# manyeyes/K2TransducerAsr

Hardware: AMD Instinct MI355X
Metric: RTFx (audio-sec/wall-sec) offline Zipformer greedy (higher is better)
Workload: dtype f32

## Files before the change

### k2transducerasr_amd/csrc/engine.cpp

```cpp
#include <cstring>
#include <thread>

#include "engine.h"
#include "lattice_ref.h"
#include "ctc_lattice_ref.h"
#include "kws_ref.h"
#include "ctc_prefix_bias_ref.h"
#include "ctc_prefix_ref.h"
#include "hotwords.h"
#include "ngram_lm.h"

#include <climits>
#include <cmath>

namespace k2hip {

namespace {
constexpr int kTailFrames = 19;
}

Engine::Engine(const std::string& weights, const char* overrides, int device) : device_(device) {
    tunables_init_from_env();
    model_.reset(new Model(weights, overrides));
    int n = 0;
// ... 233 lines not shown
    Arena& ar = *c.arena;
    const int D0 = m.cfg().dim[0];
    float* out = ar.take<float>((int64_t)B * T3 * D0);
    int64_t mark = ar.mark();
    float* a1 = ar.take<float>((int64_t)B * T1 * F0 * 8);
    conv0_swoosh(c, x, m.w("encoder_embed.conv.0.weight"), m.w("encoder_embed.conv.0.bias"), a1, B, T, F0);
    c.add_flops(0, 2.0 * B * T1 * (double)F0 * 8 * 9, 0);
    float* a2 = ar.take<float>((int64_t)B * T2 * F2 * 32);
    {
        GemmArgs g;
        g.A = a1; g.W = m.w("encoder_embed.conv.4.weight#ohwi"); g.ldw = 72; g.bias = m.w("encoder_embed.conv.4.bias");
        g.C = a2; g.ldc = 32; g.M = B * T2 * F2; g.N = 32; g.K = 72; g.act = ACT_SWOOSH_R;
        g.cv_Fout = F2; g.cv_Tout = T2; g.cv_Tin = T1; g.cv_Fin = F0; g.cv_C = 8; g.cv_st = 2; g.cv_sf = 2;
        g.seg_len = 24; g.seg_stride = F0 * 8;
        gemm(c, g);
    }
    float* a3 = ar.take<float>((int64_t)B * T3 * F3 * 128);
    {
        GemmArgs g;
        g.A = a2; g.W = m.w("encoder_embed.conv.7.weight#ohwi"); g.ldw = 288; g.bias = m.w("encoder_embed.conv.7.bias");
        g.C = a3; g.ldc = 128; g.M = B * T3 * F3; g.N = 128; g.K = 288; g.act = ACT_SWOOSH_R;
        g.cv_Fout = F3; g.cv_Tout = T3; g.cv_Tin = T2; g.cv_Fin = F2; g.cv_C = 32; g.cv_st = 1; g.cv_sf = 2;
        g.seg_len = 96; g.seg_stride = F2 * 32;
        gemm(c, g);
    }
    const int npix = B * T3 * F3;
    float* dw = ar.take<float>((int64_t)npix * 128);
    dwconv7x7(c, a3, m.w("encoder_embed.convnext.depthwise_conv.weight#kc"), m.w("encoder_embed.convnext.depthwise_conv.bias"),
              dw, B, T3, T3, 3, F3, 128);
    float* hid = ar.take<float>((int64_t)npix * 384);
    linear(c, dw, 128, m.w("encoder_embed.convnext.pointwise_conv1.weight"), m.w("encoder_embed.convnext.pointwise_conv1.bias"),
           hid, 384, npix, 128, 384, ACT_SWOOSH_L);
    linear(c, hid, 384, m.w("encoder_embed.convnext.pointwise_conv2.weight"), m.w("encoder_embed.convnext.pointwise_conv2.bias"),
           a3, 128, npix, 384, 128, ACT_NONE, a3, 128);
    float* lin = ar.take<float>((int64_t)B * T3 * D0);
    linear(c, a3, F3 * 128, m.w("encoder_embed.out.weight#fc"), m.w("encoder_embed.out.bias"), lin, D0, B * T3, F3 * 128, D0);
    biasnorm(c, lin, m.w("encoder_embed.out_norm.bias"), m.w("encoder_embed.out_norm.log_scale"), out, B * T3, D0);
    ar.rewind(mark);
    *T50 = T3;
    return out;
}

const float* Engine::pos_proj_cached(const Ctx& c, int layer, const float* pe, int pe_dim, const float* W, int rows, int ncols) {
    if (c.dry) return nullptr;
    std::lock_guard<std::mutex> lk(cache_mu_);
    const auto key = std::make_pair(layer, rows);
    auto it = pp_cache_.find(key);
// ... 68 lines not shown
    auto nonlin_attention = [&]() {
        if (site) {
            linear(c, src, D, w("nonlin_attention.in_proj.weight"), w("nonlin_attention.in_proj.bias"), hid, 3 * Hc, M, D, 3 * Hc);
            nonlin_av_out_ring(c, aw, ring(lay_.nonlin[gl]), hid, 3 * Hc, nullptr, nullptr, tmp2, B, T, KL, KLp, Hc, D);
        } else {
            GemmArgs g;
            g.A = aw; g.lda = KLp; g.sA0 = (long long)T * KLp;
            g.w_kn = 1;
            g.C = tmp2; g.ldc = Hc; g.sC0 = (long long)T * Hc;
            g.M = T; g.N = Hc; g.K = T; g.nb0 = B; g.nb1 = 1;
            if (M >= 256 && Hc % 16 == 0 && !tunables().no_glu_epilogue) {
                GemmArgs p;
                p.A = src; p.lda = D; p.W = w("nonlin_attention.in_proj.weight#glu"); p.ldw = D; p.bias = w("nonlin_attention.in_proj.bias#glu");
                p.C = hid; p.ldc = 2 * Hc; p.M = M; p.N = 3 * Hc; p.K = D; p.glu = 2; p.glu_cols = 2 * Hc;
                gemm(c, p);
                g.W = hid; g.ldw = 2 * Hc; g.sW0 = (long long)T * 2 * Hc;
                g.mul = hid + Hc; g.ldm = 2 * Hc; g.sM0 = (long long)T * 2 * Hc;
            } else {
                linear(c, src, D, w("nonlin_attention.in_proj.weight"), w("nonlin_attention.in_proj.bias"), hid, 3 * Hc, M, D, 3 * Hc);
                tanh_gate(c, hid, tmp, M, Hc);
                g.W = tmp; g.ldw = Hc; g.sW0 = (long long)T * Hc;
                g.mul = hid + 2 * Hc; g.ldm = 3 * Hc; g.sM0 = (long long)T * 3 * Hc;
            }
            gemm(c, g);
        }
        linear(c, tmp2, Hc, w("nonlin_attention.out_proj.weight"), w("nonlin_attention.out_proj.bias"), src, D, M, Hc, D, ACT_NONE, src, D);
    };
    auto self_attn = [&](int k) {
        const float *wi = wk("self_attn%d.in_proj.weight", k), *bi = wk("self_attn%d.in_proj.bias", k);
        const float *wo = wk("self_attn%d.out_proj.weight", k), *bo = wk("self_attn%d.out_proj.bias", k);
        if (vproj_fused) {
            attn_proj_av_out_ring(c, aw, ring(k == 1 ? lay_.val1[gl] : lay_.val2[gl]), src, wi, bi, wo, bo, src_alt, B, T, KL, KLp, H, vh, D);
            std::swap(src, src_alt);
            return;
        }
        linear(c, src, D, wi, bi, hid, HV, M, D, HV);
        if (site) {
            attn_av_out_ring(c, aw, ring(k == 1 ? lay_.val1[gl] : lay_.val2[gl]), hid, wo, bo, src, B, T, KL, KLp, H, vh, D);
            return;
        }
        if (attn_av_out(c, aw, hid, wo, bo, src, B, T, T, KLp, H, vh, D)) return;
        GemmArgs g;
        g.A = aw; g.lda = KLp; g.sA0 = (long long)T * KLp; g.sA1 = (long long)B * T * KLp;
        g.W = hid; g.w_kn = 1; g.ldw = HV; g.sW0 = (long long)T * HV; g.sW1 = vh;
        g.C = tmp; g.ldc = HV; g.sC0 = (long long)T * HV; g.sC1 = vh;
        g.M = T; g.N = vh; g.K = T; g.nb0 = B; g.nb1 = H;
        gemm(c, g);
// ... 1673 lines not shown
            const int ldh = I();
            float *wout = P(), *bias = P(), *x = P();
            const int B = I(), T = I(), KL = I(), Tp = I(), Hc = I(), D = I();
            nonlin_av_out_ring(c, aw, r, hid, ldh, wout, bias, x, B, T, KL, Tp, Hc, D);
        } else if (name == "attn_stream_ring" || name == "attn_stream") {
            float* qkp = P();
            const int ld = I();
            RingRef r;
            float* kcat = nullptr;
            if (name == "attn_stream_ring") r = ring(); else kcat = P();
            float* pp = P();
            const long long* plen = reinterpret_cast<const long long*>(P());
            float* aw = P();
            const int B = I(), Tc = I(), Lc = I(), KLp = I(), H = I(), ds = I(), left50 = I();
            if (kcat) attn_stream(c, qkp, ld, kcat, pp, plen, aw, B, Tc, Lc, KLp, H, ds, left50);
            else attn_stream_ring(c, qkp, ld, r, pp, plen, aw, B, Tc, Lc, KLp, H, ds, left50);
        } else if (name == "glu_causal_conv") {
            float *x2 = P(), *pool = P();
            const long long ss = L(), off = L();
            const int* slots = reinterpret_cast<const int*>(P());
            float *wc = P(), *bc = P(), *ww = P(), *bw = P(), *sc = P(), *y = P();
            const int B = I(), Tc = I(), D = I(), K = I();
            glu_causal_conv(c, x2, pool, ss, off, slots, wc, bc, ww, bw, sc, y, B, Tc, D, K);
        } else if (name == "gemm") {
            GemmArgs g;
            g.M = I(); g.N = I(); g.K = I();
            g.lda = I(); g.ldw = I(); g.ldc = I(); g.ldr = I();
            g.act = I(); g.act_cols = I(); g.w_kn = I();
            g.nb0 = I(); g.nb1 = I();
            g.sA0 = L(); g.sA1 = L(); g.sW0 = L(); g.sW1 = L(); g.sC0 = L(); g.sC1 = L(); g.sR0 = L(); g.sR1 = L();
            g.sBias0 = L();
            g.cv_Fout = I(); g.cv_Tout = I(); g.cv_Tin = I(); g.cv_Fin = I(); g.cv_C = I(); g.cv_st = I(); g.cv_sf = I();
            g.seg_len = I(); g.seg_stride = I();
            g.res_div = I(); g.act_after_res = I();
            g.glu = I(); g.glu_cols = I();
            g.ldm = I(); g.sM0 = L(); g.sM1 = L();
            g.ld_orig = I();
            const int cfg = I(), res_is_C = I();
            const long long oA = L(), oW = L(), oR = L(), oC = L(), oM = L(), oO = L();
            float *A = P(), *W = P(), *bias = P(), *res = P(), *C = P();
            const int* skip = reinterpret_cast<const int*>(P());
            float *mul = P(), *orig = P(), *scale = P();
            int* plan_out = reinterpret_cast<int*>(P());
            K2_REQUIRE(A && W && C && plan_out && buf_bytes[n_bufs - 1] >= 20, "debug_op_run gemm: A, W, C and a plan buffer of 5 ints are needed");
            K2_REQUIRE(!(res_is_C && res), "debug_op_run gemm: res_is_C takes no res buffer");
            K2_REQUIRE(oA >= 0 && oW >= 0 && oR >= 0 && oC >= 0 && oM >= 0 && oO >= 0, "debug_op_run gemm: negative offset");
            if (res_is_C) res = C;
            g.A = A + oA; g.W = W + oW; g.bias = bias; g.res = res ? res + oR : nullptr; g.C = C + oC;
            g.skip_if_zero = skip;
            g.mul = mul ? mul + oM : nullptr;
            g.byp_orig = orig ? orig + oO : nullptr; g.byp_scale = scale;
            GemmForceGuard force(cfg);
            const GemmPlan pl = plan_gemm(g, gemm_force());
            const int rep[5] = {(int)pl.family, pl.idx, pl.BM, pl.BN, pl.mode};
            K2_HIP(copy_blocking(plan_out, rep, sizeof rep, hipMemcpyHostToDevice));
            gemm(c, g);
        } else if (name == "gemm_glu_causal_conv") {
            float *x = P(), *wg = P(), *bg = P(), *pool = P();
            const long long ss = L(), off = L();
            const int* slots = reinterpret_cast<const int*>(P());
            float *wc = P(), *bc = P(), *ww = P(), *bw = P(), *sc = P(), *y = P();
            const int B = I(), Tc = I(), D = I(), K = I();
            int* entry_out = reinterpret_cast<int*>(P());
            K2_REQUIRE(entry_out && buf_bytes[n_bufs - 1] >= 4, "debug_op_run gemm_glu_causal_conv: an entry buffer of 1 int is needed");
            const int entry = glu_conv_ring_entry(B, Tc, D, K);
            K2_HIP(copy_blocking(entry_out, &entry, sizeof entry, hipMemcpyHostToDevice));
            took = gemm_glu_causal_conv(c, x, wg, bg, pool, ss, off, slots, wc, bc, ww, bw, sc, y, B, Tc, D, K);
        } else if (name == "biasnorm") {
            float *x = P(), *bias = P(), *ls = P(), *y = P();
            const int M = I(), D = I();
            biasnorm(c, x, bias, ls, y, M, D);
        } else if (name == "bypass") {
            float *orig = P(), *x = P(), *scale = P(), *y = P();
            const int M = I(), D = I();
            bypass(c, orig, x, scale, y, M, D);
        } else if (name == "biasnorm_bypass") {
            float *x = P(), *orig = P(), *nb = P(), *ls = P(), *scale = P(), *y = P();
            const int M = I(), D = I();
            biasnorm_bypass(c, x, orig, nb, ls, scale, y, M, D);
// ... 730 lines not shown
```

### k2transducerasr_amd/csrc/gemm.hip

```cpp
#include <algorithm>
#include <cmath>
#include <cstdlib>
#include <map>
#include <mutex>
#include <type_traits>

#include "act.h"
#include "kernels.h"

#pragma clang diagnostic ignored "-Winline-asm"

namespace k2hip {

typedef float f32x16 __attribute__((ext_vector_type(16)));
typedef float f32x4 __attribute__((ext_vector_type(4)));

namespace {


__device__ __forceinline__ float apply_act(float v, int act) {
    switch (act) {
        case ACT_SWOOSH_L: return swoosh_l(v);
        case ACT_SWOOSH_R: return swoosh_r(v);
        case ACT_TANH: {
// ... 481 lines not shown
            }
        }
    }

    K2_DMA_STAMP()
#pragma unroll
    for (int j = 0; j < NT; j++)
#pragma unroll
        for (int i = 0; i < MT; i++) {
            float vals[16];
#pragma unroll
            for (int r = 0; r < 16; r++) vals[r] = acc[i][j][r];
            epilogue_rows<16, Rows32>(g, vals, m0 + wr * WM + i * 32 + 4 * lh, n0 + wc * WN + j * 32 + li, C, nullptr, rres[i][j], R != nullptr,
                                      nullptr, g.bias ? g.bias + z0 * g.sBias0 : nullptr);
        }
    K2_DMA_STAMP()
    if (stamp && lane == 0) {
        stamp[62] = nstamp;
        stamp[63] = __builtin_amdgcn_s_memrealtime();
    }
#undef K2_DMA_STAMP
}

template <int BM, int BN, int WM, int WN, int NST>
__global__ __launch_bounds__(64 * (BM / WM) * (BN / WN)) void gemm_f32_mfma_pipe(GemmArgs g) {
    constexpr int BK = 32;
    constexpr int MT = WM / 32, NT = WN / 32;
    constexpr int WCOLS = BN / WN;
    constexpr int NW = (BM / WM) * (BN / WN);
    constexpr int NINST = (BM + BN) / 8;
    constexpr int IPW = NINST / NW;
    constexpr int STAGE = (BM + BN) * BK;
    constexpr int DPE = (IPW + 3) / 4;
    static_assert(NST == 3 || NST == 4, "pipe: three or four stages");
    static_assert(NINST % NW == 0, "pipe: every wave issues the same number of DMA instructions");
    static_assert((NST - 2) * IPW <= 63 && MT <= 4 && NT <= 2, "pipe: counted wait / wave tile out of range");

    if (g.skip_if_zero && *g.skip_if_zero == 0) return;
    extern __shared__ __attribute__((aligned(16))) float smem[];

    const int tid = threadIdx.x;
    const int lane = tid & 63, wave = __builtin_amdgcn_readfirstlane(tid >> 6);
    const int wr = wave / WCOLS, wc = wave % WCOLS;
    const int li = lane & 31, lh = lane >> 5;
    float* __restrict__ C = g.C;
    const float* __restrict__ R = g.res;
    int mb_, nb_;
    xcd_tile(mb_, nb_, g.xcd_panels == 1 ? 0 : g.M, g.N);
    const int m0 = mb_ * BM, n0 = nb_ * BN;
    const int nk = g.K / BK;

    unsigned long long* stamp = g.dbg ? g.dbg + ((size_t)(blockIdx.x + blockIdx.y * gridDim.x) * NW + wave) * 64 : nullptr;
    int nstamp = 0;
#define K2_PIPE_STAMP()                                                    \
    if (stamp) {  \
        if (lane == 0) stamp[nstamp] = __builtin_amdgcn_s_memtime();       \
        nstamp++;                                                          \
    }
    if (stamp && lane == 0) stamp[60] = __builtin_amdgcn_s_memrealtime();
    K2_PIPE_STAMP()

    const unsigned lds_base = (unsigned)(unsigned long long)(__attribute__((address_space(3))) char*)smem;
    unsigned voff[IPW];
    unsigned long long sb[IPW];
    unsigned mq[IPW];
#pragma unroll
    for (int q = 0; q < IPW; q++) {
        const int inst = wave + q * NW;
        const int slot = inst * 64 + lane;
        const int r = slot >> 3, cp = slot & 7;
        const int c = cp ^ ((r >> 1) & 7);
        const bool is_a = inst < BM / 8;
        const long long row = is_a ? min(m0 + r, g.M - 1) : min(n0 + (r - BM), g.N - 1);
        voff[q] = (unsigned)((row * (is_a ? g.lda : g.ldw) + 4 * c) * 4);
        const unsigned long long base = (unsigned long long)(is_a ? g.A : g.W);
        sb[q] = ((unsigned long long)(unsigned)__builtin_amdgcn_readfirstlane((int)(base >> 32)) << 32) |
                (unsigned long long)(unsigned)__builtin_amdgcn_readfirstlane((int)(unsigned)base);
        mq[q] = __builtin_amdgcn_readfirstlane(lds_base + inst * 1024);
    }

#define K2_PIPE_DMA(ST_, KT_, q_)                                                                                          \
    {                                                                                                                      \
        const unsigned long long src_ = sb[q_] + (unsigned long long)(KT_) * (BK * 4);                                    \
        asm volatile("s_add_u32 m0, %2, %3\n\ts_nop 0\n\tglobal_load_lds_dwordx4 %0, %1"                                    \
                     :                                                                                                     \
                     : "v"(voff[q_]), "s"(src_), "s"(mq[q_]), "n"((ST_) * STAGE * 4)                                       \
                     : "memory", "m0", "scc");                                                                                          \
    }
#define K2_PIPE_READ(SET_, ST_, G_)                                                                                        \
    {                                                                                                                      \
        _Pragma("unroll") for (int i = 0; i < MT; i++) fa[SET_][i] = *reinterpret_cast<const f32x4*>(ra[ST_][G_] + i * 32 * BK); \
        _Pragma("unroll") for (int j = 0; j < NT; j++) fb[SET_][j] = *reinterpret_cast<const f32x4*>(rb[ST_][G_] + j * 32 * BK); \
    }
#define K2_PIPE_FRAGS_READY(SET_) {}
#define K2_PIPE_STEP(ST_, KT_, HAS_NEXT_, DO_ISSUE_, WAIT_)                                                                \
    _Pragma("unroll") for (int gk = 0; gk < 4; gk++) {                                                                     \
        const int cu = gk & 1;                                                                                             \
        __builtin_amdgcn_sched_barrier(0);                                                                                 \
        K2_PIPE_FRAGS_READY(cu)                                                                                            \
        _Pragma("unroll") for (int e = 0; e < 4; e++) {                                                                    \
            _Pragma("unroll") for (int i = 0; i < MT; i++) _Pragma("unroll") for (int j = 0; j < NT; j++)                  \
                acc[i][j] = __builtin_amdgcn_mfma_f32_32x32x2f32(fa[cu][i][e], fb[cu][j][e], acc[i][j], 0, 0, 0);          \
            if (e == 0) {                                                                                                  \
                __builtin_amdgcn_sched_barrier(0);                                                                         \
                if (gk == 0) K2_PIPE_READ(1, ST_, 1)                                                                       \
                if (gk == 1) K2_PIPE_READ(0, ST_, 2)                                                                       \
                if (gk == 2) K2_PIPE_READ(1, ST_, 3)                                                                       \
                if (gk == 3 && (HAS_NEXT_)) K2_PIPE_READ(0, ((ST_) + 1) % NST, 0)                                          \
                __builtin_amdgcn_sched_barrier(0);                                                                         \
            }                                                                                                              \
            if (gk == 3 && (DO_ISSUE_)) {                                                                                  \
                __builtin_amdgcn_sched_barrier(0);                                                                         \
                _Pragma("unroll") for (int q = e * DPE; q < (e + 1) * DPE && q < IPW; q++)                                 \
                    K2_PIPE_DMA(((ST_) + NST - 1) % NST, (KT_) + NST - 1, q)                                               \
                __builtin_amdgcn_sched_barrier(0);                                                                         \
            }                                                                                                              \
        }                                                                                                                  \
        if (gk == 2 && (HAS_NEXT_)) {        \
            __builtin_amdgcn_sched_barrier(0);                                                                             \
            WAIT_                                                                                                          \
            __builtin_amdgcn_s_barrier();                                                                                  \
            if ((KT_) < 40) { K2_PIPE_STAMP() }                                                                            \
            __builtin_amdgcn_sched_barrier(0);                                                                             \
        }                                                                                                                  \
    }
#define K2_PIPE_WAIT_STEADY asm volatile("s_waitcnt vmcnt(%0)" ::"n"((NST - 3) * IPW) : "memory");
#define K2_PIPE_WAIT_DRAIN asm volatile("s_waitcnt vmcnt(0)" ::: "memory");

#pragma unroll
    for (int p = 0; p < NST - 1; p++)
        if (p < nk) {
#pragma unroll
            for (int q = 0; q < IPW; q++) {
                if (p == 0) K2_PIPE_DMA(0, 0, q)
                if (p == 1) K2_PIPE_DMA(1, 1, q)
                if (p == 2) K2_PIPE_DMA(2, 2, q)
            }
        }
    const int arow = wr * WM + li, brow = wc * WN + li;
    const int swa = (arow >> 1) & 7, swb = ((BM + brow) >> 1) & 7;
    const float* ra[NST][4];
    const float* rb[NST][4];
#pragma unroll
    for (int st = 0; st < NST; st++)
#pragma unroll
        for (int gk = 0; gk < 4; gk++) {
            ra[st][gk] = smem + st * STAGE + arow * BK + (((2 * gk + lh) ^ swa) << 2);
            rb[st][gk] = smem + st * STAGE + (BM + brow) * BK + (((2 * gk + lh) ^ swb) << 2);
        }

    f32x16 acc[MT][NT];
#pragma unroll
    for (int i = 0; i < MT; i++)
#pragma unroll
        for (int j = 0; j < NT; j++)
#pragma unroll
            for (int r = 0; r < 16; r++) acc[i][j][r] = 0.f;
    f32x4 fa[2][MT], fb[2][NT];
    K2_PIPE_STAMP()
    if (nk >= NST - 1) asm volatile("s_waitcnt vmcnt(%0)" ::"n"((NST - 2) * IPW) : "memory");
    else asm volatile("s_waitcnt vmcnt(0)" ::: "memory");
    __builtin_amdgcn_s_barrier();
    K2_PIPE_READ(0, 0, 0)
    K2_PIPE_STAMP()
    float rres[MT][NT][16];
    if (R) {
#pragma unroll
        for (int j = 0; j < NT; j++) {
            const int col = min(n0 + wc * WN + j * 32 + li, g.N - 1);
#pragma unroll
            for (int i = 0; i < MT; i++)
// ... 14 lines not shown
        K2_PIPE_STEP(0, kt, true, true, K2_PIPE_WAIT_STEADY)
        K2_PIPE_STEP(1, kt + 1, true, true, K2_PIPE_WAIT_STEADY)
        K2_PIPE_STEP(2, kt + 2, true, true, K2_PIPE_WAIT_STEADY)
        if (NST == 4) { K2_PIPE_STEP(NST == 4 ? 3 : 0, kt + 3, true, true, K2_PIPE_WAIT_STEADY) }
    }
#define K2_PIPE_S(j_) K2_PIPE_STEP((j_) % NST, kt + (j_), true, true, K2_PIPE_WAIT_STEADY)
#define K2_PIPE_T(j_) K2_PIPE_STEP((j_) % NST, kt + (j_), true, false, K2_PIPE_WAIT_DRAIN)
#define K2_PIPE_L(j_) K2_PIPE_STEP((j_) % NST, kt + (j_), false, false, K2_PIPE_WAIT_DRAIN)
    const int rs = nsteady - kt;
    if (NST == 3) {
        switch (rs) {
            case 0: K2_PIPE_T(0) K2_PIPE_L(1) break;
            case 1: K2_PIPE_S(0) K2_PIPE_T(1) K2_PIPE_L(2) break;
            default: K2_PIPE_S(0) K2_PIPE_S(1) K2_PIPE_T(2) K2_PIPE_L(3) break;
        }
    } else {
        switch (rs) {
            case 0: K2_PIPE_T(0) K2_PIPE_T(1) K2_PIPE_L(2) break;
            case 1: K2_PIPE_S(0) K2_PIPE_T(1) K2_PIPE_T(2) K2_PIPE_L(3) break;
            case 2: K2_PIPE_S(0) K2_PIPE_S(1) K2_PIPE_T(2) K2_PIPE_T(3) K2_PIPE_L(4) break;
            default: K2_PIPE_S(0) K2_PIPE_S(1) K2_PIPE_S(2) K2_PIPE_T(3) K2_PIPE_T(4) K2_PIPE_L(5) break;
        }
    }
#undef K2_PIPE_S
#undef K2_PIPE_T
#undef K2_PIPE_L
    K2_PIPE_STAMP()
#undef K2_PIPE_WAIT_DRAIN
#undef K2_PIPE_WAIT_STEADY
#undef K2_PIPE_STEP
#undef K2_PIPE_FRAGS_READY
#undef K2_PIPE_READ
#undef K2_PIPE_DMA

#pragma unroll
    for (int j = 0; j < NT; j++)
#pragma unroll
        for (int i = 0; i < MT; i++) {
            float vals[16];
#pragma unroll
            for (int r = 0; r < 16; r++) vals[r] = acc[i][j][r];
            epilogue_rows<16, Rows32>(g, vals, m0 + wr * WM + i * 32 + 4 * lh, n0 + wc * WN + j * 32 + li, C, nullptr, rres[i][j], R != nullptr,
                                      nullptr, g.bias, true, bias_pre[j]);
        }
    K2_PIPE_STAMP()
    if (stamp && lane == 0) {
        stamp[62] = nstamp;
        stamp[63] = __builtin_amdgcn_s_memrealtime();
    }
#undef K2_PIPE_STAMP
}

template <int BM, int BN, int WM, int WN, int NST>
__global__ __launch_bounds__(64 * (BM / WM) * (BN / WN)) void gemm_f32_mfma_p16(GemmArgs g) {
    constexpr int BK = 32;
    constexpr int MT = WM / 16, NT = WN / 16;
    constexpr int WCOLS = BN / WN;
    constexpr int NW = (BM / WM) * (BN / WN);
    constexpr int NINST = (BM + BN) / 8;
    constexpr int IPW = NINST / NW;
    constexpr int STAGE = (BM + BN) * BK;
    constexpr int DPE = (IPW + 3) / 4;
    static_assert(NST == 3, "p16: three stages");
    static_assert(NINST % NW == 0, "p16: every wave issues the same number of DMA instructions");
    static_assert(MT >= 1 && NT >= 1 && MT * NT <= 12, "p16: wave tile");

// ... 655 lines not shown
    hipLaunchKernelGGL((gemm_f32_mfma_ring<BM, BN, KS, NST, LW, PF>), grid, dim3(64 * ((BM / 32) * (BN / 32) * KS + LW + PF)), lds, ctx.stream, a);
}

template <int BM, int BN, int KS, int NST, int PF = 0>
void launch_ring_conv(const Ctx& ctx, const GemmArgs& a) {
    dim3 grid(cdiv(a.N, BN), cdiv(a.M, BM), 1);
    const int pad = a.cf_K >> 1, Kc = (a.cf_K + 1) >> 1, CH = BN / 2;
    const size_t conv_fl = (size_t)(BM / a.cf_Tc) * CH * (pad + a.cf_Tc) + (size_t)CH * (Kc | 1) + (size_t)CH * a.cf_K;
    size_t lds = sizeof(float) * std::max({(size_t)NST * KS * (BM + BN) * 32, KS > 1 ? (size_t)KS * (BM / 32) * (BN / 32) * 1024 : (size_t)0, conv_fl}) + (PF ? 256 : 0);
    static LdsAttrOnce lds_attr;
    lds_attr.ensure(gemm_f32_mfma_ring<BM, BN, KS, NST, 0, PF, true>, (int)lds);
    hipLaunchKernelGGL((gemm_f32_mfma_ring<BM, BN, KS, NST, 0, PF, true>), grid, dim3(64 * ((BM / 32) * (BN / 32) * KS + PF)), lds, ctx.stream, a);
}

template <int BM, int BN, int WM, int WN, int NST>
void launch_pipe(const Ctx& ctx, const GemmArgs& a) {
    dim3 grid(cdiv(a.N, BN), cdiv(a.M, BM), 1);
    size_t lds = sizeof(float) * NST * (BM + BN) * 32;
    static LdsAttrOnce lds_attr;
    lds_attr.ensure(gemm_f32_mfma_pipe<BM, BN, WM, WN, NST>, (int)lds);
    K2_REQUIRE((long long)a.M * a.lda < (1ll << 29) && (long long)a.N * a.ldw < (1ll << 29), "pipe: operand too large for 31-bit lane byte offsets");
    K2_REQUIRE(a.K % 32 == 0 && a.K >= 32 * (NST - 1), "pipe: K %d too short for %d stages", a.K, NST);
    hipLaunchKernelGGL((gemm_f32_mfma_pipe<BM, BN, WM, WN, NST>), grid, dim3(64 * (BM / WM) * (BN / WN)), lds, ctx.stream, a);
}

template <int BM, int BN, int WM, int WN, int NST>
void launch_p16(const Ctx& ctx, const GemmArgs& a) {
    dim3 grid(cdiv(a.N, BN), cdiv(a.M, BM), 1);
    size_t lds = sizeof(float) * NST * (BM + BN) * 32;
    static LdsAttrOnce lds_attr;
    lds_attr.ensure(gemm_f32_mfma_p16<BM, BN, WM, WN, NST>, (int)lds);
    K2_REQUIRE((long long)a.M * a.lda < (1ll << 29) && (long long)a.N * a.ldw < (1ll << 29), "p16: operand too large for 31-bit lane byte offsets");
    K2_REQUIRE(a.K % 32 == 0 && a.K >= 32 * (NST - 1) && !a.glu, "p16: K %d too short for %d stages, or a gated epilogue", a.K, NST);
    hipLaunchKernelGGL((gemm_f32_mfma_p16<BM, BN, WM, WN, NST>), grid, dim3(64 * (BM / WM) * (BN / WN)), lds, ctx.stream, a);
}

template <int BM, int BN, int WM, int WN, int BK, int MODE>
void launch_cfg(const Ctx& ctx, const GemmArgs& a) {
    constexpr int LDSK = BK + 4;
    dim3 grid(cdiv(a.N, BN), cdiv(a.M, BM), a.nb0 * a.nb1);
    size_t lds = sizeof(float) * 2 * (BM + BN) * LDSK;
    static LdsAttrOnce lds_attr;
    lds_attr.ensure(gemm_f32_mfma<BM, BN, WM, WN, BK, MODE>, (int)lds);
    hipLaunchKernelGGL((gemm_f32_mfma<BM, BN, WM, WN, BK, MODE>), grid, dim3(64 * (BM / WM) * (BN / WN)), lds, ctx.stream, a);
}

// ... 92 lines not shown
    const int entry = glu_conv_ring_entry(B, Tc, D, K);
    if (entry < 0) return false;
    const double fl = 2.0 * M * (double)N * D;
    ctx.add_flops(fl, 2.0 * M * (double)D * (K + (K + 1) / 2), 1);
    if (ctx.dry) return true;
    GemmArgs g;
    g.A = x; g.lda = D; g.W = wg; g.ldw = D; g.bias = bg; g.C = y; g.ldc = D; g.M = M; g.N = N; g.K = D;
    g.cf_pool = pool; g.cf_stride = slot_stride; g.cf_off = off; g.cf_slots = slots;
    g.cf_wc = wc; g.cf_bc = bc; g.cf_ww = ww; g.cf_bw = bw; g.cf_sc = sc; g.cf_Tc = Tc; g.cf_K = K;
    g.xcd_panels = tunables().xcd_panels;
    if (ctx.instrument) K2_HIP(hipEventRecord(ctx.next_event(), ctx.stream));
    if (ctx.instrument && ctx.gemm_log) ctx.gemm_log->push_back({M, N, D, 1, 0, 0, 64, 0.f});
    switch (entry) {
        case 16: launch_ring_conv_entry<16>(ctx, g); break;
        case 17: launch_ring_conv_entry<17>(ctx, g); break;
        case 12: launch_ring_conv_entry<12>(ctx, g); break;
        default: launch_ring_conv_entry<8>(ctx, g); break;
    }
    K2_HIP(hipGetLastError());
    if (ctx.instrument) K2_HIP(hipEventRecord(ctx.next_event(), ctx.stream));
    return true;
}

void linear(const Ctx& ctx, const float* A, int lda, const float* W, const float* bias, float* C, int ldc, int M, int K,
            int N, int act, const float* res, int ldr) {
    GemmArgs g;
    g.A = A; g.lda = lda; g.W = W; g.ldw = K; g.bias = bias; g.C = C; g.ldc = ldc;
    g.M = M; g.N = N; g.K = K; g.act = act; g.res = res; g.ldr = ldr;
    gemm(ctx, g);
}

}
```

### k2transducerasr_amd/csrc/gemm_plan.cpp

```cpp
#include "kernels.h"

namespace k2hip {

namespace {

GemmForce g_force;

bool entry(GemmFamily f, int idx, GemmPlan* p) {
    p->family = f;
    p->idx = idx;
    switch (f) {
#define X(i, bm, bn, wm, wn, bk_or_nst) case i: p->BM = bm; p->BN = bn; p->waves = (bm / wm) * (bn / wn); return true;
        case GemmFamily::REG: switch (idx) { K2_REG_TABLE(X) } return false;
        case GemmFamily::DMA: switch (idx) { K2_DMA_TABLE(X) } return false;
        case GemmFamily::PIPE: switch (idx) { K2_PIPE_TABLE(X) } return false;
        case GemmFamily::P16: switch (idx) { K2_P16_TABLE(X) } return false;
#undef X
        case GemmFamily::RING: {
            if (idx < 0 || idx >= (int)(sizeof(kRing) / sizeof(kRing[0]))) return false;
            const RingCfg& r = kRing[idx];
            p->BM = r.BM;
            p->BN = r.BN;
            p->waves = (r.BM / 32) * (r.BN / 32) * r.KS + r.LW + r.PF;
            return true;
// ... 140 lines not shown
int gemm_kind(const GemmArgs& a, const GemmPlan& p) {
    const int base = a.cv_Fout > 0 ? 1 : (a.w_kn ? 2 : 0);
    switch (p.family) {
        case GemmFamily::REG: return base;
        case GemmFamily::DMA: return base + 16;
        case GemmFamily::SKINNY3: case GemmFamily::SKINNY6: case GemmFamily::SKINNY6_8: return base + 32;
        case GemmFamily::RING: return base + 64;
        case GemmFamily::PIPE: return base + 128 + 256 * (p.BM / 32) + 4096 * (p.BN / 32);
        case GemmFamily::P16: return base + 128 + 256 * (p.BM / 32) + 4096 * (p.BN / 32) + (1 << 20);
    }
    return base;
}

int glu_conv_ring_entry(int B, int Tc, int D, int K) {
    const int M = B * Tc, N = 2 * D;
    if (Tc < 2 || 32 % Tc != 0 || D % 64 != 0 || (K != 31 && K != 15 && K != 7)) return -1;
    int e = small_ring_entry(M, N, D);
    if (e < 0) e = 8;
    const RingCfg& r = kRing[e];
    if ((long long)(r.BM / Tc) * (r.BN / 2) * (K >> 1) > 8ll * (r.BM / 32) * (r.BN / 32) * r.KS * 64) return -1;
    return e;
}

}
```

### k2transducerasr_amd/csrc/kernels.h

```cpp
#pragma once
#include "ctc_prefix_layout.h"
#include "common.h"

namespace k2hip {

#ifdef K2HIP_DEV
#define K2HIP_DEV_SWITCH(name, def) int name = def
#else
#define K2HIP_DEV_SWITCH(name, def) static constexpr int name = def
#endif
struct Tunables {
    int no_glu_epilogue = 0;
    int attn_long = 0;
    int no_fused_av = 0;
    int fused_vproj_min_t = 4;
    int no_fused_vproj = 0;
    int no_fused_conv = 0;
    int conformer_gemm_scores = 0;
    int dw7_tiled = 0;
    int dw1d_tt = 0;
    int lstm_seq = 0;
    int greedy_one_part = 0;
    int greedy_parts = 0;
    int beam_launches = 0;
// ... 78 lines not shown
    int seg_len = 0, seg_stride = 0;
    int res_div = 1;
    int act_after_res = 0;
    int glu = 0;
    int glu_cols = 0;
    const float* mul = nullptr;
    int ldm = 0;
    long long sM0 = 0, sM1 = 0;
    const float* byp_orig = nullptr;
    const float* byp_scale = nullptr;
    int ld_orig = 0;
    float* cf_pool = nullptr;
    long long cf_stride = 0, cf_off = 0;
    const int* cf_slots = nullptr;
    const float *cf_wc = nullptr, *cf_bc = nullptr, *cf_ww = nullptr, *cf_bw = nullptr, *cf_sc = nullptr;
    int cf_Tc = 0, cf_K = 0;
    unsigned long long* dbg = nullptr;
    int ablate = 0;
};
void gemm(const Ctx& ctx, const GemmArgs& a);
bool gemm_glu_causal_conv(const Ctx& ctx, const float* x, const float* wg, const float* bg, float* pool, long long slot_stride, long long off,
                          const int* slots, const float* wc, const float* bc, const float* ww, const float* bw, const float* sc, float* y, int B,
                          int Tc, int D, int K);

#define K2_PIPE_TABLE(X)                                                                                                       \
    X(0, 128, 64, 64, 32, 3) X(1, 128, 64, 32, 32, 3) X(2, 128, 128, 64, 64, 3) X(3, 128, 128, 64, 32, 3) X(4, 128, 64, 64, 32, 4)  \
    X(5, 64, 64, 32, 32, 3) X(6, 128, 128, 64, 64, 4) X(7, 64, 128, 32, 64, 3) X(8, 128, 128, 32, 32, 3) X(9, 128, 64, 32, 32, 4) \
    X(10, 64, 64, 64, 32, 3) X(11, 64, 64, 32, 64, 3) X(12, 256, 64, 64, 32, 3) X(13, 128, 32, 32, 32, 3) X(14, 128, 32, 64, 32, 3)
#define K2_P16_TABLE(X) X(0, 64, 96, 32, 48, 3) X(1, 128, 96, 64, 48, 3) X(2, 64, 192, 32, 96, 3) X(3, 32, 96, 16, 48, 3)
#define K2_RING_TABLE(X)                                                                                        \
    X(0, 128, 64, 1, 2, 0, 0) X(1, 128, 64, 1, 3, 0, 0) X(2, 128, 64, 1, 2, 0, 1) X(3, 128, 64, 1, 3, 0, 1) X(4, 128, 64, 1, 4, 0, 1)   \
    X(5, 64, 64, 1, 3, 0, 0) X(6, 64, 64, 1, 3, 0, 1) X(7, 64, 64, 1, 4, 0, 1) X(8, 64, 64, 2, 3, 0, 0) X(9, 64, 64, 2, 3, 0, 1)      \
    X(10, 64, 64, 4, 2, 0, 0) X(11, 64, 64, 4, 2, 0, 1) X(12, 32, 64, 2, 3, 0, 0) X(13, 32, 64, 4, 3, 0, 0) X(14, 32, 64, 4, 3, 0, 1)  \
    X(15, 32, 32, 4, 3, 0, 0) X(16, 32, 32, 4, 4, 0, 1) X(17, 64, 32, 4, 3, 0, 0) X(18, 128, 128, 1, 2, 0, 0) X(19, 128, 128, 1, 2, 0, 1) \
    X(20, 64, 128, 1, 3, 0, 0) X(21, 64, 128, 1, 3, 0, 1) X(22, 64, 96, 1, 3, 0, 0) X(23, 64, 96, 1, 3, 0, 1) X(24, 128, 96, 1, 2, 0, 1) \
    X(25, 128, 64, 1, 3, 2, 0) X(26, 128, 64, 1, 3, 2, 1) X(27, 128, 64, 2, 2, 0, 1) X(28, 64, 96, 2, 3, 0, 0) X(29, 64, 96, 2, 2, 0, 0) \
    X(30, 64, 96, 2, 2, 0, 1) X(31, 128, 96, 1, 3, 0, 0) X(32, 128, 96, 1, 3, 0, 1)
struct RingCfg { int BM, BN, KS, NST, LW, PF; };
#define X(i, bm, bn, ks, nst, lw, pf) {bm, bn, ks, nst, lw, pf},
constexpr RingCfg kRing[] = {K2_RING_TABLE(X)};
#undef X
#define K2_DMA_TABLE(X)                                                                                                          \
    X(0, 128, 128, 64, 32, 3) X(5, 128, 64, 32, 32, 2) X(8, 128, 64, 32, 32, 4) X(9, 64, 64, 32, 32, 2) X(10, 64, 64, 32, 32, 3) \
    X(11, 64, 96, 32, 32, 2) X(20, 32, 32, 32, 32, 4) X(21, 32, 64, 32, 32, 4)
#define K2_REG_TABLE(X)                                                                                                           \
    X(0, 128, 128, 64, 32, 32) X(1, 128, 128, 64, 32, 64) X(2, 64, 64, 32, 32, 32) X(3, 64, 64, 32, 32, 64) X(4, 128, 64, 32, 32, 64) \
    X(5, 128, 64, 32, 32, 32) X(12, 128, 32, 32, 32, 32)
enum GemmMode { MODE_PLAIN = 0, MODE_CONV = 1, MODE_WKN = 2 };

enum class GemmFamily { REG, DMA, PIPE, P16, RING, SKINNY3, SKINNY6, SKINNY6_8 };
struct GemmPlan {
    GemmFamily family = GemmFamily::REG;
    int idx = 0;
    int mode = MODE_PLAIN;
    int ablate = 0;
    int BM = 0, BN = 0, waves = 0;
};
struct GemmForce {
    enum Kind { AUTO, CFG, RING, PIPE, P16 } kind = AUTO;
    int idx = -1;
    int ablate = 0;
    bool dma = true;
};
GemmForce decode_gemm_force(int code);
GemmPlan plan_gemm(const GemmArgs& a, const GemmForce& f);
int gemm_kind(const GemmArgs& a, const GemmPlan& p);
int glu_conv_ring_entry(int B, int Tc, int D, int K);
void debug_force_gemm_cfg(int code);
GemmForce gemm_force();
struct GemmForceGuard {
    explicit GemmForceGuard(int code) { debug_force_gemm_cfg(code); }
    ~GemmForceGuard() { debug_force_gemm_cfg(-1); }
    GemmForceGuard(const GemmForceGuard&) = delete;
    GemmForceGuard& operator=(const GemmForceGuard&) = delete;
};
void linear(const Ctx& ctx, const float* A, int lda, const float* W, const float* bias, float* C, int ldc, int M, int K,
            int N, int act = ACT_NONE, const float* res = nullptr, int ldr = 0);

struct RingRef {
    float* pool = nullptr;
    long long slot_stride = 0;
    long long off = 0;
    const int* slots = nullptr;
    const int* chunks = nullptr;
};

void attn_scores_softmax(const Ctx& ctx, const float* qkp, int ld, const float* pp, float* aw, int B, int T, int Tp, int H, int qh = 32,
                         int koff0 = -1, int poff0 = -1);

bool attn_av_out(const Ctx& ctx, const float* aw, const float* v, const float* wout, const float* bias, float* x, int B, int T, int KL, int Tp,
// ... 426 lines not shown
```

Baseline: 23980.

## Route conv-embed and [K,N] attention GEMMs through the multistage DMA pipe kernel

Extends the pipelined MFMA GEMM kernel with two variants. One gathers the implicit-im2col conv A operand using segment-wrapping addresses, used for the encoder_embed conv.7 layer. The other loads a [K,N] row-major W operand batched over blockIdx.z, with a register-staged K tail and an optional multiply epilogue, used for the nonlin-attention weight×value product. Both replace the generic planner's kernels when size thresholds are met, aiming for DMA-to-LDS overlap on these shapes. The cost is extra template complexity and an extra LDS stage for the [K,N] variant.

```diff
diff --git a/k2transducerasr_amd/csrc/engine.cpp b/k2transducerasr_amd/csrc/engine.cpp
--- a/k2transducerasr_amd/csrc/engine.cpp
+++ b/k2transducerasr_amd/csrc/engine.cpp
@@ -279,7 +279,7 @@
         g.C = a3; g.ldc = 128; g.M = B * T3 * F3; g.N = 128; g.K = 288; g.act = ACT_SWOOSH_R;
         g.cv_Fout = F3; g.cv_Tout = T3; g.cv_Tin = T2; g.cv_Fin = F2; g.cv_C = 32; g.cv_st = 1; g.cv_sf = 2;
         g.seg_len = 96; g.seg_stride = F2 * 32;
-        gemm(c, g);
+        if (!gemm_conv_pipe(c, g)) gemm(c, g);
     }
     const int npix = B * T3 * F3;
     float* dw = ar.take<float>((int64_t)npix * 128);
@@ -394,7 +394,7 @@
                 g.W = tmp; g.ldw = Hc; g.sW0 = (long long)T * Hc;
                 g.mul = hid + 2 * Hc; g.ldm = 3 * Hc; g.sM0 = (long long)T * 3 * Hc;
             }
-            gemm(c, g);
+            if (!gemm_kn_pipe(c, g)) gemm(c, g);
         }
         linear(c, tmp2, Hc, w("nonlin_attention.out_proj.weight"), w("nonlin_attention.out_proj.bias"), src, D, M, Hc, D, ACT_NONE, src, D);
     };
@@ -2114,7 +2114,7 @@
             float *wc = P(), *bc = P(), *ww = P(), *bw = P(), *sc = P(), *y = P();
             const int B = I(), Tc = I(), D = I(), K = I();
             glu_causal_conv(c, x2, pool, ss, off, slots, wc, bc, ww, bw, sc, y, B, Tc, D, K);
-        } else if (name == "gemm") {
+        } else if (name == "gemm" || name == "gemm_conv_pipe" || name == "gemm_kn_pipe") {
             GemmArgs g;
             g.M = I(); g.N = I(); g.K = I();
             g.lda = I(); g.ldw = I(); g.ldc = I(); g.ldr = I();
@@ -2130,6 +2130,8 @@
             g.ld_orig = I();
             const int cfg = I(), res_is_C = I();
             const long long oA = L(), oW = L(), oR = L(), oC = L(), oM = L(), oO = L();
+            const bool conv_pipe = name == "gemm_conv_pipe", kn_pipe = name == "gemm_kn_pipe";
+            const int force_form = conv_pipe || kn_pipe ? I() : 0;
             float *A = P(), *W = P(), *bias = P(), *res = P(), *C = P();
             const int* skip = reinterpret_cast<const int*>(P());
             float *mul = P(), *orig = P(), *scale = P();
@@ -2142,11 +2144,17 @@
             g.skip_if_zero = skip;
             g.mul = mul ? mul + oM : nullptr;
             g.byp_orig = orig ? orig + oO : nullptr; g.byp_scale = scale;
-            GemmForceGuard force(cfg);
-            const GemmPlan pl = plan_gemm(g, gemm_force());
-            const int rep[5] = {(int)pl.family, pl.idx, pl.BM, pl.BN, pl.mode};
-            K2_HIP(copy_blocking(plan_out, rep, sizeof rep, hipMemcpyHostToDevice));
-            gemm(c, g);
+            if (conv_pipe) {
+                took = gemm_conv_pipe(c, g, force_form != 0);
+            } else if (kn_pipe) {
+                took = gemm_kn_pipe(c, g, force_form != 0);
+            } else {
+                GemmForceGuard force(cfg);
+                const GemmPlan pl = plan_gemm(g, gemm_force());
+                const int rep[5] = {(int)pl.family, pl.idx, pl.BM, pl.BN, pl.mode};
+                K2_HIP(copy_blocking(plan_out, rep, sizeof rep, hipMemcpyHostToDevice));
+                gemm(c, g);
+            }
         } else if (name == "gemm_glu_causal_conv") {
             float *x = P(), *wg = P(), *bg = P(), *pool = P();
             const long long ss = L(), off = L();
diff --git a/k2transducerasr_amd/csrc/gemm.hip b/k2transducerasr_amd/csrc/gemm.hip
--- a/k2transducerasr_amd/csrc/gemm.hip
+++ b/k2transducerasr_amd/csrc/gemm.hip
@@ -527,7 +527,7 @@
 #undef K2_DMA_STAMP
 }
 
-template <int BM, int BN, int WM, int WN, int NST>
+template <int BM, int BN, int WM, int WN, int NST, bool CONV = false, bool KN = false>
 __global__ __launch_bounds__(64 * (BM / WM) * (BN / WN)) void gemm_f32_mfma_pipe(GemmArgs g) {
     constexpr int BK = 32;
     constexpr int MT = WM / 32, NT = WN / 32;
@@ -540,6 +540,10 @@
     static_assert(NST == 3 || NST == 4, "pipe: three or four stages");
     static_assert(NINST % NW == 0, "pipe: every wave issues the same number of DMA instructions");
     static_assert((NST - 2) * IPW <= 63 && MT <= 4 && NT <= 2, "pipe: counted wait / wave tile out of range");
+    constexpr int QA = (BM / 8) / NW;
+    static_assert(!(CONV || KN) || (BM / 8) % NW == 0, "pipe, conv gather / [K,N]: the A / W split of a wave's DMA instructions must not depend on the wave");
+    static_assert(!KN || (BN == 64 && NT == 1 && !CONV && (BM * 8) % (64 * NW) == 0 && (BK * 16) % (64 * NW) == 0), "pipe, [K,N]: 64-column tiles");
+    constexpr int NSTL = KN ? NST + 1 : NST;
 
     if (g.skip_if_zero && *g.skip_if_zero == 0) return;
     extern __shared__ __attribute__((aligned(16))) float smem[];
@@ -548,12 +552,16 @@
     const int lane = tid & 63, wave = __builtin_amdgcn_readfirstlane(tid >> 6);
     const int wr = wave / WCOLS, wc = wave % WCOLS;
     const int li = lane & 31, lh = lane >> 5;
-    float* __restrict__ C = g.C;
+    const int z0 = KN ? (int)blockIdx.z : 0;
+    float* __restrict__ C = KN ? g.C + z0 * g.sC0 : g.C;
     const float* __restrict__ R = g.res;
+    const float* __restrict__ Ab = KN ? g.A + z0 * g.sA0 : g.A;
+    const float* __restrict__ Wb = KN ? g.W + z0 * g.sW0 : g.W;
     int mb_, nb_;
     xcd_tile(mb_, nb_, g.xcd_panels == 1 ? 0 : g.M, g.N);
     const int m0 = mb_ * BM, n0 = nb_ * BN;
     const int nk = g.K / BK;
+    [[maybe_unused]] const bool has_tail = KN && (g.K % BK) != 0;
 
     unsigned long long* stamp = g.dbg ? g.dbg + ((size_t)(blockIdx.x + blockIdx.y * gridDim.x) * NW + wave) * 64 : nullptr;
     int nstamp = 0;
@@ -577,16 +585,57 @@
         const int c = cp ^ ((r >> 1) & 7);
         const bool is_a = inst < BM / 8;
         const long long row = is_a ? min(m0 + r, g.M - 1) : min(n0 + (r - BM), g.N - 1);
-        voff[q] = (unsigned)((row * (is_a ? g.lda : g.ldw) + 4 * c) * 4);
-        const unsigned long long base = (unsigned long long)(is_a ? g.A : g.W);
+        if (KN && !is_a) {
+            const int k = 4 * (inst - BM / 8) + (lane >> 4), cc = (lane & 15) ^ (((k >> 2) & 1) << 3);
+            voff[q] = (unsigned)(((long long)k * g.ldw + min(n0 + 4 * cc, g.N - 4)) * 4);
+        } else if (CONV && is_a) {
+            const int rw = (int)row, f = rw % g.cv_Fout, bt = rw / g.cv_Fout, t = bt % g.cv_Tout, b = bt / g.cv_Tout;
+            voff[q] = (unsigned)(((((long long)b * g.cv_Tin + (long long)t * g.cv_st) * g.cv_Fin + (long long)f * g.cv_sf) * g.cv_C + 4 * c) * 4);
+        } else {
+            voff[q] = (unsigned)((row * (is_a ? g.lda : g.ldw) + 4 * c) * 4);
+        }
+        const unsigned long long base = (unsigned long long)(is_a ? Ab : Wb);
         sb[q] = ((unsigned long long)(unsigned)__builtin_amdgcn_readfirstlane((int)(base >> 32)) << 32) |
                 (unsigned long long)(unsigned)__builtin_amdgcn_readfirstlane((int)(unsigned)base);
         mq[q] = __builtin_amdgcn_readfirstlane(lds_base + inst * 1024);
     }
-
+    const unsigned long long wstep = KN ? (unsigned long long)g.ldw * (BK * 4) : (unsigned long long)(BK * 4);
+    constexpr int NTHR = 64 * NW, TPA = KN ? BM * 8 / NTHR : 1, TPW = KN ? BK * 16 / NTHR : 1;
+    [[maybe_unused]] float4 ta[TPA], tw[TPW];
+    [[maybe_unused]] bool oka[TPA], okw[TPW];
+    if constexpr (KN) {
+        if (has_tail) {
+            const int kt0 = nk * BK, Kp = (g.K + 3) & ~3;
+#pragma unroll
+            for (int p = 0; p < TPA; p++) {
+                const int sl = tid + NTHR * p, r = sl >> 3, k = kt0 + 4 * ((sl & 7) ^ ((r >> 1) & 7));
+                oka[p] = k < Kp;
+                ta[p] = *reinterpret_cast<const float4*>(Ab + (long long)min(m0 + r, g.M - 1) * g.lda + (oka[p] ? k : Kp - 4));
+            }
+#pragma unroll
+            for (int p = 0; p < TPW; p++) {
+                const int sl = tid + NTHR * p, k = sl >> 4, cc = (sl & 15) ^ (((k >> 2) & 1) << 3);
+                okw[p] = kt0 + k < g.K;
+                tw[p] = *reinterpret_cast<const float4*>(Wb + (long long)(okw[p] ? kt0 + k : g.K - 1) * g.ldw + min(n0 + 4 * cc, g.N - 4));
+            }
+        }
+    }
+
+    unsigned long long a_run = sb[0];
+    const int seg_steps = CONV ? g.seg_len / BK : 0;
+    const unsigned long long seg_wrap = CONV ? (unsigned long long)(long long)(g.seg_stride - g.seg_len + BK) * 4 : 0;
+    int seg_left = seg_steps;
+#define K2_PIPE_ADVANCE()                                    \
+    if (CONV) {                                              \
+        const bool wrap_ = --seg_left == 0;                  \
+        a_run += wrap_ ? seg_wrap : (unsigned long long)(BK * 4); \
+        seg_left = wrap_ ? seg_steps : seg_left;             \
+    }
 #define K2_PIPE_DMA(ST_, KT_, q_)                                                                                          \
     {                                                                                                                      \
-        const unsigned long long src_ = sb[q_] + (unsigned long long)(KT_) * (BK * 4);                                    \
+        const unsigned long long src_ = CONV && (q_) < QA ? a_run                                                          \
+                                        : KN && (q_) >= QA ? sb[q_] + (unsigned long long)(KT_) * wstep                    \
+                                                           : sb[q_] + (unsigned long long)(KT_) * (BK * 4);                \
         asm volatile("s_add_u32 m0, %2, %3\n\ts_nop 0\n\tglobal_load_lds_dwordx4 %0, %1"                                    \
                      :                                                                                                     \
                      : "v"(voff[q_]), "s"(src_), "s"(mq[q_]), "n"((ST_) * STAGE * 4)                                       \
@@ -595,7 +644,11 @@
 #define K2_PIPE_READ(SET_, ST_, G_)                                                                                        \
     {                                                                                                                      \
         _Pragma("unroll") for (int i = 0; i < MT; i++) fa[SET_][i] = *reinterpret_cast<const f32x4*>(ra[ST_][G_] + i * 32 * BK); \
-        _Pragma("unroll") for (int j = 0; j < NT; j++) fb[SET_][j] = *reinterpret_cast<const f32x4*>(rb[ST_][G_] + j * 32 * BK); \
+        if constexpr (KN) {                                                                                                \
+            _Pragma("unroll") for (int e_ = 0; e_ < 4; e_++) fb[SET_][0][e_] = rb[ST_][G_][e_ * BN];                       \
+        } else {                                                                                                           \
+            _Pragma("unroll") for (int j = 0; j < NT; j++) fb[SET_][j] = *reinterpret_cast<const f32x4*>(rb[ST_][G_] + j * 32 * BK); \
+        }                                                                                                                  \
     }
 #define K2_PIPE_FRAGS_READY(SET_) {}
 #define K2_PIPE_STEP(ST_, KT_, HAS_NEXT_, DO_ISSUE_, WAIT_)                                                                \
@@ -612,12 +665,16 @@
                 if (gk == 1) K2_PIPE_READ(0, ST_, 2)                                                                       \
                 if (gk == 2) K2_PIPE_READ(1, ST_, 3)                                                                       \
                 if (gk == 3 && (HAS_NEXT_)) K2_PIPE_READ(0, ((ST_) + 1) % NST, 0)                                          \
+                if constexpr (KN) {                              \
+                    if (gk == 3 && !(HAS_NEXT_) && (ST_) != NST && has_tail) K2_PIPE_READ(0, NST, 0)                       \
+                }                                                                                                          \
                 __builtin_amdgcn_sched_barrier(0);                                                                         \
             }                                                                                                              \
             if (gk == 3 && (DO_ISSUE_)) {                                                                                  \
                 __builtin_amdgcn_sched_barrier(0);                                                                         \
                 _Pragma("unroll") for (int q = e * DPE; q < (e + 1) * DPE && q < IPW; q++)                                 \
                     K2_PIPE_DMA(((ST_) + NST - 1) % NST, (KT_) + NST - 1, q)                                               \
+                if (e == 3) K2_PIPE_ADVANCE()                                                                              \
                 __builtin_amdgcn_sched_barrier(0);                                                                         \
             }                                                                                                              \
         }                                                                                                                  \
@@ -641,17 +698,29 @@
                 if (p == 1) K2_PIPE_DMA(1, 1, q)
                 if (p == 2) K2_PIPE_DMA(2, 2, q)
             }
-        }
+            K2_PIPE_ADVANCE()
+        }
+    if constexpr (KN) {
+        if (has_tail) {
+            float* ts = smem + NST * STAGE;
+#pragma unroll
+            for (int p = 0; p < TPA; p++) *reinterpret_cast<float4*>(ts + (tid + NTHR * p) * 4) = sel4(oka[p], ta[p]);
+#pragma unroll
+            for (int p = 0; p < TPW; p++) *reinterpret_cast<float4*>(ts + BM * BK + (tid + NTHR * p) * 4) = sel4(okw[p], tw[p]);
+            asm volatile("s_waitcnt lgkmcnt(0)" ::: "memory");
+        }
+    }
     const int arow = wr * WM + li, brow = wc * WN + li;
     const int swa = (arow >> 1) & 7, swb = ((BM + brow) >> 1) & 7;
-    const float* ra[NST][4];
-    const float* rb[NST][4];
-#pragma unroll
-    for (int st = 0; st < NST; st++)
+    const float* ra[NSTL][4];
+    const float* rb[NSTL][4];
+#pragma unroll
+    for (int st = 0; st < NSTL; st++)
 #pragma unroll
         for (int gk = 0; gk < 4; gk++) {
             ra[st][gk] = smem + st * STAGE + arow * BK + (((2 * gk + lh) ^ swa) << 2);
-            rb[st][gk] = smem + st * STAGE + (BM + brow) * BK + (((2 * gk + lh) ^ swb) << 2);
+            if (KN) rb[st][gk] = smem + st * STAGE + BM * BK + (8 * gk + 4 * lh) * BN + (brow ^ (lh << 5));
+            else rb[st][gk] = smem + st * STAGE + (BM + brow) * BK + (((2 * gk + lh) ^ swb) << 2);
         }
 
     f32x16 acc[MT][NT];
@@ -712,6 +781,9 @@
             default: K2_PIPE_S(0) K2_PIPE_S(1) K2_PIPE_S(2) K2_PIPE_T(3) K2_PIPE_T(4) K2_PIPE_L(5) break;
         }
     }
+    if constexpr (KN) {
+        if (has_tail) { K2_PIPE_STEP(NST, 0, false, false, K2_PIPE_WAIT_DRAIN) }
+    }
 #undef K2_PIPE_S
 #undef K2_PIPE_T
 #undef K2_PIPE_L
@@ -722,6 +794,7 @@
 #undef K2_PIPE_FRAGS_READY
 #undef K2_PIPE_READ
 #undef K2_PIPE_DMA
+#undef K2_PIPE_ADVANCE
 
 #pragma unroll
     for (int j = 0; j < NT; j++)
@@ -731,7 +804,7 @@
 #pragma unroll
             for (int r = 0; r < 16; r++) vals[r] = acc[i][j][r];
             epilogue_rows<16, Rows32>(g, vals, m0 + wr * WM + i * 32 + 4 * lh, n0 + wc * WN + j * 32 + li, C, nullptr, rres[i][j], R != nullptr,
-                                      nullptr, g.bias, true, bias_pre[j]);
+                                      KN && g.mul ? g.mul + z0 * g.sM0 : nullptr, g.bias, true, bias_pre[j]);
         }
     K2_PIPE_STAMP()
     if (stamp && lane == 0) {
@@ -1433,6 +1506,26 @@
     K2_REQUIRE((long long)a.M * a.lda < (1ll << 29) && (long long)a.N * a.ldw < (1ll << 29), "pipe: operand too large for 31-bit lane byte offsets");
     K2_REQUIRE(a.K % 32 == 0 && a.K >= 32 * (NST - 1), "pipe: K %d too short for %d stages", a.K, NST);
     hipLaunchKernelGGL((gemm_f32_mfma_pipe<BM, BN, WM, WN, NST>), grid, dim3(64 * (BM / WM) * (BN / WN)), lds, ctx.stream, a);
+}
+
+template <int BM, int BN, int WM, int WN, int NST>
+void launch_pipe_conv(const Ctx& ctx, const GemmArgs& a) {
+    dim3 grid(cdiv(a.N, BN), cdiv(a.M, BM), 1);
+    size_t lds = sizeof(float) * NST * (BM + BN) * 32;
+    static LdsAttrOnce lds_attr;
+    lds_attr.ensure(gemm_f32_mfma_pipe<BM, BN, WM, WN, NST, true>, (int)lds);
+    K2_REQUIRE(a.K % 32 == 0 && a.K >= 32 * (NST - 1) && a.seg_len % 32 == 0, "pipe, conv gather: K %d / segments of %d floats", a.K, a.seg_len);
+    hipLaunchKernelGGL((gemm_f32_mfma_pipe<BM, BN, WM, WN, NST, true>), grid, dim3(64 * (BM / WM) * (BN / WN)), lds, ctx.stream, a);
+}
+
+template <int BM, int BN, int WM, int WN, int NST>
+void launch_pipe_kn(const Ctx& ctx, const GemmArgs& a) {
+    dim3 grid(cdiv(a.N, BN), cdiv(a.M, BM), a.nb0);
+    size_t lds = sizeof(float) * (NST + 1) * (BM + BN) * 32;
+    static LdsAttrOnce lds_attr;
+    lds_attr.ensure(gemm_f32_mfma_pipe<BM, BN, WM, WN, NST, false, true>, (int)lds);
+    K2_REQUIRE(a.K >= 32 * (NST - 1) && a.nb1 == 1 && a.N % 4 == 0, "pipe, [K,N]: K %d too short for %d stages, or not one batch dimension", a.K, NST);
+    hipLaunchKernelGGL((gemm_f32_mfma_pipe<BM, BN, WM, WN, NST, false, true>), grid, dim3(64 * (BM / WM) * (BN / WN)), lds, ctx.stream, a);
 }
 
 template <int BM, int BN, int WM, int WN, int NST>
@@ -1571,6 +1664,42 @@
     return true;
 }
 
+bool gemm_conv_pipe(const Ctx& ctx, const GemmArgs& a, bool force) {
+    if (!gemm_conv_pipe_takes(a, force)) return false;
+    const double fl = 2.0 * a.M * (double)a.N * a.K;
+    ctx.add_flops(fl, 0.0, 1);
+    if (ctx.dry) return true;
+    if (ctx.instrument) K2_HIP(hipEventRecord(ctx.next_event(), ctx.stream));
+    GemmArgs b = a;
+    b.ablate = 0;
+    b.xcd_panels = tunables().xcd_panels;
+    GemmPlan p;
+    p.family = GemmFamily::PIPE; p.idx = 1; p.BM = 128; p.BN = 64; p.waves = 8;
+    launch_pipe_conv<128, 64, 32, 32, 3>(ctx, b);
+    K2_HIP(hipGetLastError());
+    if (ctx.instrument && ctx.gemm_log) ctx.gemm_log->push_back({a.M, a.N, a.K, 1, a.act, a.res != nullptr, gemm_kind(a, p), 0.f});
+    if (ctx.instrument) K2_HIP(hipEventRecord(ctx.next_event(), ctx.stream));
+    return true;
+}
+
+bool gemm_kn_pipe(const Ctx& ctx, const GemmArgs& a, bool force) {
+    if (!gemm_kn_pipe_takes(a, force)) return false;
+    const double fl = 2.0 * a.M * (double)a.N * a.K * a.nb0;
+    ctx.add_flops(fl, 0.0, 1);
+    if (ctx.dry) return true;
+    if (ctx.instrument) K2_HIP(hipEventRecord(ctx.next_event(), ctx.stream));
+    GemmArgs b = a;
+    b.ablate = 0;
+    b.xcd_panels = tunables().xcd_panels;
+    GemmPlan p;
+    p.family = GemmFamily::PIPE; p.idx = 5; p.BM = 64; p.BN = 64; p.waves = 4;
+    launch_pipe_kn<64, 64, 32, 32, 3>(ctx, b);
+    K2_HIP(hipGetLastError());
+    if (ctx.instrument && ctx.gemm_log) ctx.gemm_log->push_back({a.M, a.N, a.K, a.nb0, a.act, a.res != nullptr, gemm_kind(a, p), 0.f});
+    if (ctx.instrument) K2_HIP(hipEventRecord(ctx.next_event(), ctx.stream));
+    return true;
+}
+
 void linear(const Ctx& ctx, const float* A, int lda, const float* W, const float* bias, float* C, int ldc, int M, int K,
             int N, int act, const float* res, int ldr) {
     GemmArgs g;
diff --git a/k2transducerasr_amd/csrc/gemm_plan.cpp b/k2transducerasr_amd/csrc/gemm_plan.cpp
--- a/k2transducerasr_amd/csrc/gemm_plan.cpp
+++ b/k2transducerasr_amd/csrc/gemm_plan.cpp
@@ -186,4 +186,23 @@
     return e;
 }
 
-}
+bool gemm_conv_pipe_takes(const GemmArgs& a, bool force) {
+    if (a.cv_Fout <= 0 || a.cv_Tout <= 0 || a.w_kn || a.nb0 * a.nb1 != 1) return false;
+    if (a.seg_len <= 0 || a.seg_len % 32 != 0 || a.K % 32 != 0 || a.K < 64) return false;
+    if (a.cv_C % 4 != 0 || a.seg_stride % 4 != 0 || a.ldw % 4 != 0) return false;
+    if (a.mul || a.glu || a.res_div != 1) return false;
+    const long long streams = cdiv((long long)a.M, (long long)a.cv_Tout * a.cv_Fout);
+    if (streams * a.cv_Tin * a.cv_Fin * a.cv_C >= (1ll << 29) || (long long)a.N * a.ldw >= (1ll << 29)) return false;
+    return force || a.M >= kConvPipeMinRows;
+}
+
+bool gemm_kn_pipe_takes(const GemmArgs& a, bool force) {
+    if (!a.w_kn || a.cv_Fout > 0 || a.nb1 != 1 || a.nb0 < 1) return false;
+    const int Kp = (a.K + 3) & ~3;
+    if (a.N < 4 || a.N % 4 != 0 || a.K < 64 || a.lda % 4 != 0 || a.lda < Kp || a.ldw % 4 != 0 || a.sA0 % 4 != 0 || a.sW0 % 4 != 0) return false;
+    if (a.bias || a.res || a.glu || a.res_div != 1) return false;
+    if ((long long)a.M * a.lda >= (1ll << 29) || (long long)a.K * a.ldw >= (1ll << 29)) return false;
+    return force || a.K >= kKnPipeMinT;
+}
+
+}
diff --git a/k2transducerasr_amd/csrc/kernels.h b/k2transducerasr_amd/csrc/kernels.h
--- a/k2transducerasr_amd/csrc/kernels.h
+++ b/k2transducerasr_amd/csrc/kernels.h
@@ -124,6 +124,8 @@
 bool gemm_glu_causal_conv(const Ctx& ctx, const float* x, const float* wg, const float* bg, float* pool, long long slot_stride, long long off,
                           const int* slots, const float* wc, const float* bc, const float* ww, const float* bw, const float* sc, float* y, int B,
                           int Tc, int D, int K);
+bool gemm_conv_pipe(const Ctx& ctx, const GemmArgs& a, bool force = false);
+bool gemm_kn_pipe(const Ctx& ctx, const GemmArgs& a, bool force = false);
 
 #define K2_PIPE_TABLE(X)                                                                                                       \
     X(0, 128, 64, 64, 32, 3) X(1, 128, 64, 32, 32, 3) X(2, 128, 128, 64, 64, 3) X(3, 128, 128, 64, 32, 3) X(4, 128, 64, 64, 32, 4)  \
@@ -168,6 +170,10 @@
 GemmPlan plan_gemm(const GemmArgs& a, const GemmForce& f);
 int gemm_kind(const GemmArgs& a, const GemmPlan& p);
 int glu_conv_ring_entry(int B, int Tc, int D, int K);
+constexpr int kConvPipeMinRows = 8192;
+bool gemm_conv_pipe_takes(const GemmArgs& a, bool force);
+constexpr int kKnPipeMinT = 96;
+bool gemm_kn_pipe_takes(const GemmArgs& a, bool force);
 void debug_force_gemm_cfg(int code);
 GemmForce gemm_force();
 struct GemmForceGuard {
```

Measured after the change: 24060 (median of 6 runs). About the same (+0.3%).
